# databricks/spark-deep-learning

Measured on AMD Instinct MI355X. Metric: images/sec, higher is better.
Workload: dtype bf16; 1 GPU; model=resnet50, global_batch=512, image=224, parallelism=dp1

## Files before the change

sparkdl/models/resnet.py:

```python

import torch
import torch.nn as nn

from sparkdl.ops import BatchNormAct2d, Conv1x1


class Bottleneck(nn.Module):
    expansion = 4

    def __init__(self, cin, width, stride=1):
        super().__init__()
        cout = width * self.expansion
        self.conv1 = Conv1x1(cin, width)
        self.bn1 = BatchNormAct2d(width, relu=True)
        self.conv2 = nn.Conv2d(width, width, 3, stride=stride, padding=1,
                               bias=False)
        self.bn2 = BatchNormAct2d(width, relu=True)
        self.conv3 = Conv1x1(width, cout)
        self.bn3 = BatchNormAct2d(cout, relu=True)
        if stride != 1 or cin != cout:
            self.down_conv = Conv1x1(cin, cout, stride=stride)
            self.down_bn = BatchNormAct2d(cout, relu=False)
        else:
            self.down_conv = None

    def forward(self, x):
        if self.down_conv is not None:
            idn = self.down_bn(self.down_conv(x))
        else:
            idn = x
        out = self.bn1(self.conv1(x))
        out = self.bn2(self.conv2(out))
        return self.bn3(self.conv3(out), residual=idn)


class ResNet50(nn.Module):
    LAYERS = (3, 4, 6, 3)

    def __init__(self, num_classes=1000):
        super().__init__()
        self.stem_conv = nn.Conv2d(3, 64, 7, stride=2, padding=3,
                                   bias=False)
        self.stem_bn = BatchNormAct2d(64, relu=True)
        self.stem_pool = nn.MaxPool2d(3, stride=2, padding=1)
        cin = 64
        stages = []
        for i, blocks in enumerate(self.LAYERS):
            width = 64 * (2 ** i)
            stride = 1 if i == 0 else 2
            layer = []
            for b in range(blocks):
                layer.append(Bottleneck(cin, width, stride if b == 0 else 1))
                cin = width * Bottleneck.expansion
            stages.append(nn.Sequential(*layer))
        self.stages = nn.Sequential(*stages)
        self.pool = nn.AdaptiveAvgPool2d(1)
        self.fc = nn.Linear(2048, num_classes)

        for m in self.modules():
            if isinstance(m, nn.Conv2d):
                nn.init.kaiming_normal_(m.weight, mode="fan_out",
                                        nonlinearity="relu")
        for m in self.modules():
            if isinstance(m, Bottleneck):
                nn.init.zeros_(m.bn3.weight)

    def forward(self, x):
        x = self.stem_pool(self.stem_bn(self.stem_conv(x)))
        x = self.stages(x)
        x = self.pool(x).flatten(1)
        return self.fc(x)
```

sparkdl/ops/__init__.py:

```python

_EXT = None
_EXT_ERR = None


def ext():
    global _EXT, _EXT_ERR
    if _EXT is None and _EXT_ERR is None:
        try:
            from sparkdl import _C
            _EXT = _C
        except ImportError as e:
            _EXT_ERR = e
    if _EXT is None:
        raise RuntimeError(
            "sparkdl._C HIP extension is not built. Run "
            "`python setup.py build_ext --inplace` (gfx950). "
            "Original error: %s" % _EXT_ERR)
    return _EXT


def has_ext():
    try:
        ext()
        return True
    except RuntimeError:
        return False


from sparkdl.ops.functional import (
    layer_norm, bias_gelu, batch_norm_act, layer_norm_ref, bias_gelu_ref,
    flash_attention, flash_attention_packed, masked_attention_ref,
    seqlens_from_mask,
)
from sparkdl.ops.modules import (
    LayerNorm, Linear, LinearGelu, Conv1x1, BatchNormAct2d,
    convert_bf16_training,
)
from sparkdl.ops.optim import FusedAdamW, FusedSGD
```

sparkdl/ops/csrc/batchnorm.hip:

```cpp

#include "common.hip.h"
#include "kernels.h"

namespace {

constexpr int kBlock = 256;
constexpr int kVec = 8;
constexpr int kUnroll = 2;
constexpr int kFoldFloats = kBlock * 2 * kVec;
constexpr int kFinCh = 4;


__device__ __forceinline__ void bn_store_pair(
    float* p, int cols, const float (&a)[kVec], const float (&b)[kVec]) {
  *(float4v*)(p) = float4v{a[0], a[1], a[2], a[3]};
  *(float4v*)(p + 4) = float4v{a[4], a[5], a[6], a[7]};
  *(float4v*)(p + cols) = float4v{b[0], b[1], b[2], b[3]};
  *(float4v*)(p + cols + 4) = float4v{b[4], b[5], b[6], b[7]};
}

__device__ __forceinline__ void bn_block_fold(
    float* lds, float (&a)[kVec], float (&b)[kVec], int rpb, int row_off,
    int lane_col, int cols, float* __restrict__ slab_row) {
  const bool active = row_off < rpb;
  float* mine = lds + (size_t)row_off * 2 * cols + lane_col;
  if (active) bn_store_pair(mine, cols, a, b);
  int s = 1;
  while (s < rpb) s <<= 1;
  int n = rpb;
  for (s >>= 1; s >= 1; s >>= 1) {
    __syncthreads();
    if (row_off < s && row_off + s < n) {
      const float* peer = mine + (size_t)s * 2 * cols;
      const float4v pa0 = *(const float4v*)(peer);
      const float4v pa1 = *(const float4v*)(peer + 4);
      const float4v pb0 = *(const float4v*)(peer + cols);
      const float4v pb1 = *(const float4v*)(peer + cols + 4);
#pragma unroll
      for (int j = 0; j < 4; ++j) {
        a[j] += pa0[j];
        a[j + 4] += pa1[j];
        b[j] += pb0[j];
        b[j + 4] += pb1[j];
      }
      if (s > 1) bn_store_pair(mine, cols, a, b);
    }
    n = min(n, s);
  }
  if (row_off == 0) bn_store_pair(slab_row + lane_col, cols, a, b);
}

__device__ __forceinline__ void bn_slab_sum(
    const float* __restrict__ slab, int G, int cols, int blk, float* red,
    float& sum_a, float& sum_b) {
  const int c = blk * kFinCh + threadIdx.x % kFinCh;
  float sa = 0.f, sb = 0.f;
#pragma unroll 4
  for (int g = threadIdx.x / kFinCh; g < G; g += kBlock / kFinCh) {
    const float* row = slab + (size_t)g * 2 * cols;
    sa += row[c];
    sb += row[cols + c];
  }
#pragma unroll
  for (int off = kFinCh; off < WAVE; off <<= 1) {
    sa += __shfl_xor(sa, off, WAVE);
    sb += __shfl_xor(sb, off, WAVE);
  }
  const int lane = threadIdx.x % WAVE;
  const int wid = threadIdx.x / WAVE;
  if (lane < kFinCh) {
    red[wid * 2 * kFinCh + lane] = sa;
    red[wid * 2 * kFinCh + kFinCh + lane] = sb;
  }
  __syncthreads();
  sum_a = 0.f;
  sum_b = 0.f;
  if (threadIdx.x < kFinCh) {
#pragma unroll
    for (int w = 0; w < kBlock / WAVE; ++w) {
      sum_a += red[w * 2 * kFinCh + threadIdx.x];
      sum_b += red[w * 2 * kFinCh + kFinCh + threadIdx.x];
    }
  }
}

__device__ __forceinline__ int bn_fin_block() {
  const int nb = gridDim.x;
  if (nb % 8) return blockIdx.x;
  return (blockIdx.x % 8) * (nb / 8) + blockIdx.x / 8;
}

template <int U>
__global__ __launch_bounds__(kBlock) void bn_stats_k(
// ... 16 lines not shown
        v[u] = *(const short8*)(x + (r + u * stride) * cols + lane_col);
#pragma unroll
      for (int u = 0; u < U; ++u) {
#pragma unroll
        for (int j = 0; j < kVec; ++j) {
          const float f = bf2f(v[u][j]);
          s[j] += f;
          ss[j] += f * f;
        }
      }
    }
    for (; r < rows; r += stride) {
      const short8 v = *(const short8*)(x + r * cols + lane_col);
#pragma unroll
      for (int j = 0; j < kVec; ++j) {
        const float f = bf2f(v[j]);
        s[j] += f;
        ss[j] += f * f;
      }
    }
  }
  bn_block_fold(lds, s, ss, rpb, row_off, lane_col, cols,
                slab + (size_t)blockIdx.x * 2 * cols);
}

__global__ __launch_bounds__(kBlock) void bn_finalize_k(
    const float* __restrict__ slab, int G, const float* __restrict__ gamma,
    const float* __restrict__ beta, float* __restrict__ running_mean,
    float* __restrict__ running_var, float* __restrict__ save_mean,
    float* __restrict__ save_rstd, float* __restrict__ scale,
    float* __restrict__ shift, long long rows, int cols, float momentum,
    float eps, int training) {
  __shared__ float red[kBlock / WAVE * 2 * kFinCh];
  float sum = 0.f, sumsq = 0.f;
  const int blk = bn_fin_block();
  if (training) bn_slab_sum(slab, G, cols, blk, red, sum, sumsq);
  if (threadIdx.x >= kFinCh) return;
  const int c = blk * kFinCh + threadIdx.x;
  float mean, rstd;
  if (training) {
    mean = sum / rows;
    const float var = fmaxf(sumsq / rows - mean * mean, 0.f);
    rstd = rsqrtf(var + eps);
    const float unbiased = rows > 1 ? var * rows / (rows - 1) : var;
    running_mean[c] += momentum * (mean - running_mean[c]);
    running_var[c] += momentum * (unbiased - running_var[c]);
    save_mean[c] = mean;
    save_rstd[c] = rstd;
  } else {
    mean = running_mean[c];
    rstd = rsqrtf(running_var[c] + eps);
    save_mean[c] = mean;
    save_rstd[c] = rstd;
  }
  const float sc = gamma[c] * rstd;
  scale[c] = sc;
  shift[c] = beta[c] - mean * sc;
}

template <bool RELU, bool RES>
__global__ __launch_bounds__(kBlock) void bn_apply_k(
    const short* __restrict__ x, const short* __restrict__ res,
    const float* __restrict__ scale, const float* __restrict__ shift,
    short* __restrict__ y, unsigned char* __restrict__ mask,
    long long rows, int cols) {
  const int tpr = cols / kVec;
  const int rpb = kBlock / min(tpr, kBlock);
  const int lane_col = (threadIdx.x % tpr) * kVec;
  const int row_off = threadIdx.x / tpr;
  if (row_off >= rpb) return;
  const float4v sc0 = *(const float4v*)(scale + lane_col);
  const float4v sc1 = *(const float4v*)(scale + lane_col + 4);
  const float4v sh0 = *(const float4v*)(shift + lane_col);
  const float4v sh1 = *(const float4v*)(shift + lane_col + 4);

  for (long long r = (long long)blockIdx.x * rpb + row_off; r < rows;
       r += (long long)gridDim.x * rpb) {
    const long long base = r * cols + lane_col;
    const short8 v = *(const short8*)(x + base);
    short8 o;
    unsigned char mbits = 0;
#pragma unroll
    for (int j = 0; j < kVec; ++j) {
      float f = bf2f(v[j]) * (j < 4 ? sc0[j] : sc1[j - 4]) +
                (j < 4 ? sh0[j] : sh1[j - 4]);
      if (RES) f += bf2f(res[base + j]);
      if (RELU) {
        if (f > 0.f) mbits |= (unsigned char)(1u << j);
        f = fmaxf(f, 0.f);
      }
      o[j] = f2bf(f);
    }
    *(short8*)(y + base) = o;
    if (RELU) mask[(r * cols + lane_col) / kVec] = mbits;
  }
}


template <bool RELU, int U>
__global__ __launch_bounds__(kBlock) void bn_bwd_reduce_k(
    const short* __restrict__ x, const unsigned char* __restrict__ mask,
    const short* __restrict__ dy, const float* __restrict__ save_mean,
    const float* __restrict__ save_rstd, float* __restrict__ slab,
    long long rows, int cols) {
  __shared__ __attribute__((aligned(16))) float lds[kFoldFloats];
  const int tpr = cols / kVec;
  const int rpb = kBlock / min(tpr, kBlock);
  const int lane_col = (threadIdx.x % tpr) * kVec;
  const int row_off = threadIdx.x / tpr;

  float s1[kVec] = {0.f}, s2[kVec] = {0.f};
  if (row_off < rpb) {
    const float4v m0 = *(const float4v*)(save_mean + lane_col);
    const float4v m1 = *(const float4v*)(save_mean + lane_col + 4);
    const float4v r0 = *(const float4v*)(save_rstd + lane_col);
    const float4v r1 = *(const float4v*)(save_rstd + lane_col + 4);
    auto accum = [&](const short8& xv, const short8& dv,
                     unsigned char mbits) {
#pragma unroll
      for (int j = 0; j < kVec; ++j) {
        float d = bf2f(dv[j]);
        if (RELU && !(mbits & (1u << j))) d = 0.f;
        const float mean = j < 4 ? m0[j] : m1[j - 4];
        const float rstd = j < 4 ? r0[j] : r1[j - 4];
        const float xh = (bf2f(xv[j]) - mean) * rstd;
        s1[j] += d;
        s2[j] += d * xh;
      }
    };
    const long long stride = (long long)gridDim.x * rpb;
    long long r = (long long)blockIdx.x * rpb + row_off;
    for (; r + (U - 1) * stride < rows; r += U * stride) {
      short8 xv[U], dv[U];
      unsigned char mb[U];
#pragma unroll
      for (int u = 0; u < U; ++u) {
        const long long base = (r + u * stride) * cols + lane_col;
        xv[u] = *(const short8*)(x + base);
        dv[u] = *(const short8*)(dy + base);
        mb[u] = 0xffu;
        if (RELU) mb[u] = mask[base / kVec];
      }
#pragma unroll
      for (int u = 0; u < U; ++u) accum(xv[u], dv[u], mb[u]);
    }
    for (; r < rows; r += stride) {
      const long long base = r * cols + lane_col;
      const short8 xv = *(const short8*)(x + base);
      const short8 dv = *(const short8*)(dy + base);
      unsigned char mbits = 0xffu;
      if (RELU) mbits = mask[base / kVec];
      accum(xv, dv, mbits);
    }
  }
  bn_block_fold(lds, s1, s2, rpb, row_off, lane_col, cols,
                slab + (size_t)blockIdx.x * 2 * cols);
}

__global__ __launch_bounds__(kBlock) void bn_bwd_finalize_k(
    const float* __restrict__ slab, int G, const float* __restrict__ gamma,
    const float* __restrict__ save_rstd, float* __restrict__ dgamma,
    float* __restrict__ dbeta, float* __restrict__ c1,
    float* __restrict__ c2, float* __restrict__ c3, long long rows,
    int cols, int training) {
  __shared__ float red[kBlock / WAVE * 2 * kFinCh];
  float sum_dym, sum_dymxh;
  const int blk = bn_fin_block();
  bn_slab_sum(slab, G, cols, blk, red, sum_dym, sum_dymxh);
  if (threadIdx.x >= kFinCh) return;
  const int c = blk * kFinCh + threadIdx.x;
  dgamma[c] = sum_dymxh;
  dbeta[c] = sum_dym;
  c1[c] = gamma[c] * save_rstd[c];
  if (training) {
    c2[c] = sum_dym / rows;
    c3[c] = sum_dymxh / rows;
  } else {
    c2[c] = 0.f;
    c3[c] = 0.f;
  }
}

template <bool RELU, bool RES>
__global__ __launch_bounds__(kBlock) void bn_bwd_apply_k(
    const short* __restrict__ x, const unsigned char* __restrict__ mask,
    const short* __restrict__ dy, const float* __restrict__ save_mean,
    const float* __restrict__ save_rstd, const float* __restrict__ c1,
    const float* __restrict__ c2, const float* __restrict__ c3,
    short* __restrict__ dx, short* __restrict__ dres, long long rows,
    int cols) {
  const int tpr = cols / kVec;
  const int rpb = kBlock / min(tpr, kBlock);
  const int lane_col = (threadIdx.x % tpr) * kVec;
  const int row_off = threadIdx.x / tpr;
  if (row_off >= rpb) return;
  const float4v m0 = *(const float4v*)(save_mean + lane_col);
  const float4v m1 = *(const float4v*)(save_mean + lane_col + 4);
  const float4v r0 = *(const float4v*)(save_rstd + lane_col);
  const float4v r1 = *(const float4v*)(save_rstd + lane_col + 4);
  const float4v a0 = *(const float4v*)(c1 + lane_col);
  const float4v a1 = *(const float4v*)(c1 + lane_col + 4);
  const float4v b0 = *(const float4v*)(c2 + lane_col);
  const float4v b1 = *(const float4v*)(c2 + lane_col + 4);
  const float4v g0 = *(const float4v*)(c3 + lane_col);
  const float4v g1 = *(const float4v*)(c3 + lane_col + 4);

  for (long long r = (long long)blockIdx.x * rpb + row_off; r < rows;
       r += (long long)gridDim.x * rpb) {
    const long long base = r * cols + lane_col;
    const short8 xv = *(const short8*)(x + base);
    const short8 dv = *(const short8*)(dy + base);
    unsigned char mbits = 0xffu;
    if (RELU) mbits = mask[base / kVec];
    short8 odx, odr;
#pragma unroll
    for (int j = 0; j < kVec; ++j) {
      float d = bf2f(dv[j]);
      if (RELU && !(mbits & (1u << j))) d = 0.f;
      const float mean = j < 4 ? m0[j] : m1[j - 4];
      const float rstd = j < 4 ? r0[j] : r1[j - 4];
      const float xh = (bf2f(xv[j]) - mean) * rstd;
      const float k1 = j < 4 ? a0[j] : a1[j - 4];
      const float k2 = j < 4 ? b0[j] : b1[j - 4];
      const float k3 = j < 4 ? g0[j] : g1[j - 4];
      odx[j] = f2bf(k1 * (d - k2 - xh * k3));
      if (RES) odr[j] = f2bf(d);
    }
    *(short8*)(dx + base) = odx;
    if (RES) *(short8*)(dres + base) = odr;
  }
}

int bn_grid(long long rows, int cols) {
  const int tpr = cols / kVec;
  const int rpb = kBlock / min(tpr, kBlock);
  long long blocks = (rows + rpb - 1) / rpb;
  return (int)min(blocks, 2048LL);
}

}

int bn_reduce_blocks(long long rows, int cols) {
  const int tpr = cols / kVec;
  const int rpb = kBlock / min(tpr, kBlock);
  const long long row_blocks = (rows + rpb - 1) / rpb;
  const long long g = max(256LL, min(512LL, rows / 64));
  return (int)max(1LL, min(row_blocks, g));
}

long long bn_scratch_floats(long long rows, int cols) {
  return (long long)bn_reduce_blocks(rows, cols) * 2 * cols + 3LL * cols;
}

void launch_bn_fwd(const short* x, const short* res, const float* gamma,
                   const float* beta, float* running_mean,
                   float* running_var, float* save_mean, float* save_rstd,
                   float* scratch, short* y, unsigned char* mask,
                   long long rows, int cols, float momentum, float eps,
                   bool training, bool relu, hipStream_t stream) {
  const int grid = bn_grid(rows, cols);
  const int G = bn_reduce_blocks(rows, cols);
  if (training)
    hipLaunchKernelGGL(bn_stats_k<kUnroll>, dim3(G), dim3(kBlock), 0,
                       stream, x, scratch, rows, cols);
  float* scale = scratch + (size_t)G * 2 * cols;
  float* shift = scale + cols;
  hipLaunchKernelGGL(bn_finalize_k, dim3(cols / kFinCh), dim3(kBlock), 0,
                     stream, scratch, G, gamma, beta, running_mean,
                     running_var, save_mean, save_rstd, scale, shift, rows,
                     cols, momentum, eps, (int)training);
  auto ap = relu ? (res ? bn_apply_k<true, true> : bn_apply_k<true, false>)
                 : (res ? bn_apply_k<false, true>
                        : bn_apply_k<false, false>);
  hipLaunchKernelGGL(ap, dim3(grid), dim3(kBlock), 0, stream, x, res,
                     scale, shift, y, mask, rows, cols);
}

void launch_bn_bwd(const short* x, const unsigned char* mask,
                   const short* dy, const float* gamma,
                   const float* save_mean, const float* save_rstd,
                   float* scratch, float* dgamma, float* dbeta, short* dx,
                   short* dres, long long rows, int cols, bool training,
                   bool relu, hipStream_t stream) {
  const int grid = bn_grid(rows, cols);
  const int G = bn_reduce_blocks(rows, cols);
  auto rk = relu ? bn_bwd_reduce_k<true, kUnroll>
                 : bn_bwd_reduce_k<false, kUnroll>;
  hipLaunchKernelGGL(rk, dim3(G), dim3(kBlock), 0, stream, x, mask, dy,
                     save_mean, save_rstd, scratch, rows, cols);
  float* c1 = scratch + (size_t)G * 2 * cols;
  float* c2 = c1 + cols;
  float* c3 = c2 + cols;
  hipLaunchKernelGGL(bn_bwd_finalize_k, dim3(cols / kFinCh), dim3(kBlock),
                     0, stream, scratch, G, gamma, save_rstd, dgamma, dbeta,
                     c1, c2, c3, rows, cols, (int)training);
  auto ak = relu ? (dres ? bn_bwd_apply_k<true, true>
                         : bn_bwd_apply_k<true, false>)
                 : (dres ? bn_bwd_apply_k<false, true>
                         : bn_bwd_apply_k<false, false>);
  hipLaunchKernelGGL(ak, dim3(grid), dim3(kBlock), 0, stream, x, mask, dy,
                     save_mean, save_rstd, c1, c2, c3, dx, dres, rows,
                     cols);
}
```

sparkdl/ops/csrc/bindings.cpp:

```cpp

#include <torch/extension.h>
#include <ATen/hip/impl/HIPStreamMasqueradingAsCUDA.h>
#include <ATen/hip/impl/HIPGuardImplMasqueradingAsCUDA.h>

#include <cmath>
#include <vector>

#include "kernels.h"

namespace {

using DeviceGuard = c10::hip::HIPGuardMasqueradingAsCUDA;

hipStream_t cur_stream() {
  return c10::hip::getCurrentHIPStreamMasqueradingAsCUDA().stream();
}

#define CHECK_BF16_CUDA(t)                                            \
  TORCH_CHECK((t).is_cuda(), #t " must be on GPU");                   \
  TORCH_CHECK((t).scalar_type() == at::kBFloat16, #t " must be bf16");\
  TORCH_CHECK((t).is_contiguous(), #t " must be contiguous")

#define CHECK_F32_CUDA(t)                                             \
  TORCH_CHECK((t).is_cuda(), #t " must be on GPU");                   \
// ... 103 lines not shown
      dgamma.data_ptr<float>(), dbeta.data_ptr<float>(), ws_rows, cols,
      cur_stream());
  return {dx, dgamma, dbeta};
}


std::vector<at::Tensor> bn_fwd(const at::Tensor& x,
                               const c10::optional<at::Tensor>& res,
                               const at::Tensor& gamma,
                               const at::Tensor& beta,
                               at::Tensor running_mean,
                               at::Tensor running_var, double momentum,
                               double eps, bool training, bool relu) {
  CHECK_BF16_CUDA(x);
  CHECK_F32_CUDA(gamma);
  CHECK_F32_CUDA(beta);
  DeviceGuard guard(x.device());
  const int cols = (int)x.size(-1);
  const long long rows = x.numel() / cols;
  TORCH_CHECK(cols % 8 == 0 && cols <= 2048,
              "bn_fwd requires cols%8==0 and cols<=2048 (NHWC channels)");
  const short* res_ptr = nullptr;
  if (res.has_value()) {
    CHECK_BF16_CUDA(res.value());
    TORCH_CHECK(res->sizes() == x.sizes());
    res_ptr = bf_ptr(res.value());
  }
  auto f32 = x.options().dtype(at::kFloat);
  auto y = at::empty_like(x);
  auto save_mean = at::empty({cols}, f32);
  auto save_rstd = at::empty({cols}, f32);
  auto scratch = at::empty({bn_scratch_floats(rows, cols)}, f32);
  at::Tensor mask;
  unsigned char* mask_ptr = nullptr;
  if (relu) {
    mask = at::empty({rows * cols / 8}, x.options().dtype(at::kByte));
    mask_ptr = mask.data_ptr<unsigned char>();
  } else {
    mask = at::empty({0}, x.options().dtype(at::kByte));
  }
  launch_bn_fwd(bf_ptr(x), res_ptr, gamma.data_ptr<float>(),
                beta.data_ptr<float>(), running_mean.data_ptr<float>(),
                running_var.data_ptr<float>(), save_mean.data_ptr<float>(),
                save_rstd.data_ptr<float>(), scratch.data_ptr<float>(),
                bf_ptr_mut(y), mask_ptr, rows, cols, (float)momentum,
                (float)eps, training, relu, cur_stream());
  return {y, save_mean, save_rstd, mask};
}

std::vector<at::Tensor> bn_bwd(const at::Tensor& x,
                               const at::Tensor& mask,
                               const at::Tensor& dy,
                               const at::Tensor& gamma,
                               const at::Tensor& save_mean,
                               const at::Tensor& save_rstd, bool training,
                               bool relu, bool needs_dres) {
  CHECK_BF16_CUDA(x);
  CHECK_BF16_CUDA(dy);
  CHECK_F32_CUDA(gamma);
  DeviceGuard guard(x.device());
  const int cols = (int)x.size(-1);
  const long long rows = x.numel() / cols;
  TORCH_CHECK(!relu || mask.numel() == rows * cols / 8,
              "relu backward needs the forward's activation mask");
  auto f32 = x.options().dtype(at::kFloat);
  auto dx = at::empty_like(x);
  auto dgamma = at::empty({cols}, f32);
  auto dbeta = at::empty({cols}, f32);
  auto scratch = at::empty({bn_scratch_floats(rows, cols)}, f32);
  at::Tensor dres;
  short* dres_ptr = nullptr;
  if (needs_dres) {
    dres = at::empty_like(x);
    dres_ptr = bf_ptr_mut(dres);
  }
  launch_bn_bwd(bf_ptr(x),
                relu ? mask.data_ptr<unsigned char>() : nullptr,
                bf_ptr(dy), gamma.data_ptr<float>(),
                save_mean.data_ptr<float>(), save_rstd.data_ptr<float>(),
                scratch.data_ptr<float>(), dgamma.data_ptr<float>(),
                dbeta.data_ptr<float>(), bf_ptr_mut(dx), dres_ptr, rows,
                cols, training, relu, cur_stream());
  if (needs_dres) return {dx, dgamma, dbeta, dres};
  return {dx, dgamma, dbeta};
}


at::Tensor bias_gelu_fwd(const at::Tensor& x, const at::Tensor& bias) {
  CHECK_BF16_CUDA(x);
  CHECK_F32_CUDA(bias);
  DeviceGuard guard(x.device());
  const int cols = (int)x.size(-1);
  const long long rows = x.numel() / cols;
  TORCH_CHECK(bias.numel() == cols);
  auto y = at::empty_like(x);
  launch_bias_gelu_fwd(bf_ptr(x), bias.data_ptr<float>(), bf_ptr_mut(y),
                       rows, cols, cur_stream());
  return y;
}

std::vector<at::Tensor> bias_gelu_bwd(const at::Tensor& x,
                                      const at::Tensor& bias,
                                      const at::Tensor& dy) {
  CHECK_BF16_CUDA(x);
  CHECK_BF16_CUDA(dy);
  CHECK_F32_CUDA(bias);
  DeviceGuard guard(x.device());
  const int cols = (int)x.size(-1);
  const long long rows = x.numel() / cols;
  TORCH_CHECK(cols <= 16384, "bias_gelu_bwd LDS partials support cols<=16384");
  auto dx = at::empty_like(x);
  auto dbias = at::zeros({cols}, x.options().dtype(at::kFloat));
  launch_bias_gelu_bwd(bf_ptr(x), bias.data_ptr<float>(), bf_ptr(dy),
                       bf_ptr_mut(dx), dbias.data_ptr<float>(), rows, cols,
                       cur_stream());
  return {dx, dbias};
}


std::vector<at::Tensor> gemm_bias_act(const at::Tensor& A,
                                      const at::Tensor& W,
                                      const c10::optional<at::Tensor>& bias,
                                      int64_t act, bool save_z) {
  CHECK_BF16_CUDA(A);
  CHECK_BF16_CUDA(W);
  TORCH_CHECK(A.dim() == 2 && W.dim() == 2 && A.size(1) == W.size(1));
  const int M = (int)A.size(0), K = (int)A.size(1), N = (int)W.size(0);
  TORCH_CHECK(gemm_bias_act_supported(M, N, K),
              "gemm_bias_act requires K % 64 == 0");
  const float* bias_ptr = nullptr;
  if (bias.has_value()) {
    CHECK_F32_CUDA(bias.value());
    TORCH_CHECK(bias->numel() == N);
    bias_ptr = bias->data_ptr<float>();
  }
  DeviceGuard guard(A.device());
  auto C = at::empty({M, N}, A.options());
  at::Tensor Z;
  short* z_ptr = nullptr;
  if (save_z && act != 0) {
    Z = at::empty({M, N}, A.options());
    z_ptr = bf_ptr_mut(Z);
  }
  launch_gemm_bias_act(bf_ptr(A), bf_ptr(W), bias_ptr, bf_ptr_mut(C),
                       z_ptr, M, N, K, (int)act, cur_stream());
  if (z_ptr) return {C, Z};
  return {C};
}

at::Tensor gemm_stream(const at::Tensor& A, const at::Tensor& W) {
  CHECK_BF16_CUDA(A);
  CHECK_BF16_CUDA(W);
  TORCH_CHECK(A.dim() == 2 && W.dim() == 2 && A.size(1) == W.size(1));
  const long long M = A.size(0);
  const int K = (int)A.size(1), N = (int)W.size(0);
  TORCH_CHECK(gemm_stream_supported(M, N, K),
              "gemm_stream requires K in {64,128,256} and N % 64 == 0");
  DeviceGuard guard(A.device());
  auto C = at::empty({M, N}, A.options());
  launch_gemm_stream(bf_ptr(A), bf_ptr(W), bf_ptr_mut(C), M, N, K,
                     cur_stream());
  return C;
}


static const long long* seed_ptr(const c10::optional<at::Tensor>& seed) {
// ... 161 lines not shown
}

at::Tensor wgrad_splitk(const at::Tensor& dZ, const at::Tensor& X) {
  CHECK_BF16_CUDA(dZ);
  CHECK_BF16_CUDA(X);
  TORCH_CHECK(dZ.dim() == 2 && X.dim() == 2 && dZ.size(0) == X.size(0));
  const long long M = dZ.size(0);
  const int N = (int)dZ.size(1), K = (int)X.size(1);
  TORCH_CHECK(wgrad_splitk_supported(M, N, K),
              "wgrad_splitk requires N%256==0, K%128==0, M%64==0");
  DeviceGuard guard(dZ.device());
  auto dW = at::empty({N, K}, dZ.options().dtype(at::kFloat));
  launch_wgrad_splitk(bf_ptr(dZ), bf_ptr(X), dW.data_ptr<float>(), M, N,
                      K, cur_stream());
  return dW;
}

at::Tensor transpose_bf16(const at::Tensor& X) {
  CHECK_BF16_CUDA(X);
  TORCH_CHECK(X.dim() == 2 && X.is_contiguous());
  DeviceGuard guard(X.device());
  const int R = (int)X.size(0), C = (int)X.size(1);
  auto Y = at::empty({C, R}, X.options());
  launch_transpose_bf16(bf_ptr(X), bf_ptr_mut(Y), R, C, cur_stream());
  return Y;
}


at::Tensor gbt_histogram(const at::Tensor& B, const at::Tensor& g,
                         const at::Tensor& h, const at::Tensor& row_list,
                         const at::Tensor& bmap, int64_t n_nodes) {
  TORCH_CHECK(B.is_cuda() && B.scalar_type() == at::kByte &&
              B.is_contiguous());
  CHECK_F32_CUDA(g);
  CHECK_F32_CUDA(h);
  TORCH_CHECK(row_list.is_cuda() && row_list.scalar_type() == at::kInt);
  TORCH_CHECK(bmap.is_cuda() && bmap.scalar_type() == at::kInt &&
              bmap.size(-1) == 4);
  DeviceGuard guard(B.device());
  const int F = (int)B.size(1);
  TORCH_CHECK(F % 8 == 0, "feature dim must be padded to a multiple of 8");
  auto hist = at::zeros({n_nodes, F, 256, 2},
                        B.options().dtype(at::kFloat));
  launch_gbt_histogram(
      B.data_ptr<unsigned char>(), g.data_ptr<float>(),
      h.data_ptr<float>(), row_list.data_ptr<int>(),
      reinterpret_cast<const int4*>(bmap.data_ptr<int>()),
      (int)(bmap.numel() / 4), F, hist.data_ptr<float>(), cur_stream());
  return hist;
}

}

PYBIND11_MODULE(TORCH_EXTENSION_NAME, m) {
  m.doc() = "sparkdl MI355X-native kernels (gfx950)";
  m.def("fused_adamw_", &fused_adamw_, "Fused multi-tensor AdamW step");
  m.def("fused_sgd_", &fused_sgd_, "Fused multi-tensor SGD step");
  m.def("zero_grads_", &zero_grads_, "Zero all grads in a chunk table");
  m.def("gemm_bias_act", &gemm_bias_act, "MFMA GEMM + bias(+GELU) (N6)");
  m.def("transpose_bf16", &transpose_bf16, "bf16 2D transpose (dgrad W^T)");
  m.def("gemm_stream", &gemm_stream,
        "Streaming tall-skinny GEMM (1x1 convs)");
  m.def("wgrad_splitk", &wgrad_splitk,
        "Split-M wgrad GEMM (tr_b16 fragment path)");
  m.def("attn_fwd", &attn_fwd, "Flash attention fwd (D=64, bf16)",
        py::arg("q"), py::arg("k"), py::arg("v"), py::arg("dropout_p"),
        py::arg("seed"), py::arg("seqlens") = py::none());
  m.def("attn_bwd", &attn_bwd, "Flash attention bwd (dQ/dK/dV)",
        py::arg("q"), py::arg("k"), py::arg("v"), py::arg("dO"),
        py::arg("lse"), py::arg("drow"), py::arg("dropout_p"),
        py::arg("seed"), py::arg("seqlens") = py::none());
  m.def("attn_fwd_packed", &attn_fwd_packed,
        "Flash attention fwd over the packed qkv buffer", py::arg("qkv"),
        py::arg("dropout_p"), py::arg("seed"),
        py::arg("seqlens") = py::none());
  m.def("attn_bwd_packed", &attn_bwd_packed,
        "Flash attention bwd -> packed dqkv", py::arg("qkv"),
        py::arg("dO"), py::arg("lse"), py::arg("drow"),
        py::arg("dropout_p"), py::arg("seed"),
        py::arg("seqlens") = py::none());
  m.def("gbt_histogram", &gbt_histogram, "GBT g/h histogram (N7)");
  m.def("bn_fwd", &bn_fwd, "Fused BatchNorm(+add)(+ReLU) fwd (bf16 NHWC)");
  m.def("bn_bwd", &bn_bwd, "Fused BatchNorm(+add)(+ReLU) bwd (bf16 NHWC)");
  m.def("layernorm_fwd", &layernorm_fwd, "LayerNorm forward (bf16)");
  m.def("layernorm_bwd", &layernorm_bwd, "LayerNorm backward (bf16)");
  m.def("bias_gelu_fwd", &bias_gelu_fwd, "Fused bias+GELU forward (bf16)");
  m.def("bias_gelu_bwd", &bias_gelu_bwd, "Fused bias+GELU backward (bf16)");
  m.attr("_chunk_elems") = kOptChunk;
}
```

sparkdl/ops/csrc/kernels.h:

```cpp
#pragma once

#include <hip/hip_runtime.h>
#include <cstdint>

struct TensorChunk {
  float* p;
  const float* g;
  float* m;
  float* v;
  long long n;
  short* pl;
};

constexpr int kOptChunk = 16384;

void launch_fused_adamw(const TensorChunk* chunks, const int2* bmap,
                        int nblocks, float lr, float beta1, float beta2,
                        float eps, float weight_decay,
                        long long* step_counter, float* coeffs,
                        hipStream_t stream);

void launch_fused_sgd(const TensorChunk* chunks, const int2* bmap,
                      int nblocks, float lr, float momentum,
                      float weight_decay, bool nesterov, bool first_step,
                      hipStream_t stream);

void launch_layernorm_fwd(const short* x, const float* gamma,
                          const float* beta, short* y, float* save_mean,
                          float* save_rstd, int rows, int cols, float eps,
                          hipStream_t stream);

void launch_layernorm_bwd(const short* x, const short* dy,
                          const float* gamma, const float* save_mean,
                          const float* save_rstd, short* dx,
                          float* dgamma_part, float* dbeta_part,
                          int part_rows, int rows, int cols,
                          hipStream_t stream);

int layernorm_bwd_part_rows(int rows);

void launch_layernorm_reduce_parts(const float* dgamma_part,
                                   const float* dbeta_part, float* dgamma,
                                   float* dbeta, int part_rows, int cols,
                                   hipStream_t stream);

void launch_bias_gelu_fwd(const short* x, const float* bias, short* y,
                          long long rows, int cols, hipStream_t stream);

void launch_bias_gelu_bwd(const short* x, const float* bias,
                          const short* dy, short* dx, float* dbias,
                          long long rows, int cols, hipStream_t stream);

int bn_reduce_blocks(long long rows, int cols);
long long bn_scratch_floats(long long rows, int cols);

void launch_bn_fwd(const short* x, const short* res, const float* gamma,
                   const float* beta, float* running_mean,
                   float* running_var, float* save_mean, float* save_rstd,
                   float* scratch, short* y, unsigned char* mask,
                   long long rows, int cols, float momentum, float eps,
                   bool training, bool relu, hipStream_t stream);

void launch_bn_bwd(const short* x, const unsigned char* mask,
                   const short* dy, const float* gamma,
                   const float* save_mean, const float* save_rstd,
                   float* scratch, float* dgamma, float* dbeta, short* dx,
                   short* dres, long long rows, int cols, bool training,
                   bool relu, hipStream_t stream);

void launch_gemm_bias_act(const short* A, const short* W,
                          const float* bias, short* C, short* Z, int M,
                          int N, int K, int act, hipStream_t stream);
bool gemm_bias_act_supported(int M, int N, int K);

void launch_gemm_stream(const short* A, const short* W, short* C,
                        long long M, int N, int K, hipStream_t stream);
bool gemm_stream_supported(long long M, int N, int K);

void launch_wgrad_splitk(const short* dZ, const short* X, float* dW,
                         long long M, int N, int K, hipStream_t stream);
bool wgrad_splitk_supported(long long M, int N, int K);

void launch_transpose_bf16(const short* X, short* Y, int R, int C,
                           hipStream_t stream);

void launch_attn_pretranspose(const short* X, short* T, int BH, int S,
                              int H, int rs, hipStream_t stream);
void launch_attn_fwd(const short* Q, const short* K, const short* VT,
                     short* O, float* LSE, const long long* seed, int BH,
                     int S, int H, int rs, int ors, float dropout_p,
                     const int* seqlens, hipStream_t stream);
void launch_attn_bwd(const short* Q, const short* K, const short* V,
                     const short* dO, const short* QT, const short* DOT,
                     const short* KT, const float* LSE, const float* Drow,
                     short* dQ, short* dK, short* dV,
                     const long long* seed, int BH, int S, int H, int rs,
                     int ors, int grs, float dropout_p,
                     const int* seqlens, hipStream_t stream);

void launch_gbt_histogram(const unsigned char* B, const float* g,
                          const float* h, const int* row_list,
                          const int4* bmap, int nblocks, int F,
                          float* hist, hipStream_t stream);

void launch_zero_grads(const TensorChunk* chunks, const int2* bmap,
                       int nblocks, hipStream_t stream);
```

sparkdl/ops/functional.py:

```python

import os

import torch

import sparkdl.ops as _ops



def layer_norm_ref(x, gamma, beta, eps=1e-5):
    xf = x.float()
    out = torch.nn.functional.layer_norm(
        xf, (x.shape[-1],), gamma.float(), beta.float(), eps)
    return out.to(x.dtype)


def bias_gelu_ref(x, bias):
    return torch.nn.functional.gelu(
        x.float() + bias.float(), approximate="none").to(x.dtype)


def masked_attention_ref(q, k, v, seq_lens, dropout_p=0.0):
    S, d = q.shape[-2], q.shape[-1]
    qf, kf, vf = q.float(), k.float(), v.float()
    lens = torch.as_tensor(seq_lens, device=q.device).clamp(0, S)
# ... 39 lines not shown
        C = _ops.ext()
        x = x.contiguous()
        y, mean, rstd = C.layernorm_fwd(x, gamma, beta, eps)
        ctx.save_for_backward(x, gamma, mean, rstd)
        return y

    @staticmethod
    def backward(ctx, dy):
        C = _ops.ext()
        x, gamma, mean, rstd = ctx.saved_tensors
        dx, dgamma, dbeta = C.layernorm_bwd(
            x, dy.contiguous(), gamma, mean, rstd)
        return dx, dgamma, dbeta, None


class _BiasGeluFn(torch.autograd.Function):
    @staticmethod
    def forward(ctx, x, bias):
        C = _ops.ext()
        x = x.contiguous()
        ctx.save_for_backward(x, bias)
        return C.bias_gelu_fwd(x, bias)

    @staticmethod
    def backward(ctx, dy):
        C = _ops.ext()
        x, bias = ctx.saved_tensors
        dx, dbias = C.bias_gelu_bwd(x, bias, dy.contiguous())
        return dx, dbias


def _to_nhwc(t):
    return t.permute(0, 2, 3, 1).contiguous(memory_format=torch.contiguous_format)


def _from_nhwc(t):
    return t.permute(0, 3, 1, 2)


class _BNReLUFn(torch.autograd.Function):
    @staticmethod
    def forward(ctx, x, residual, gamma, beta, running_mean, running_var,
                momentum, eps, training, relu):
        C = _ops.ext()
        xp = _to_nhwc(x)
        rp = _to_nhwc(residual) if residual is not None else None
        y, mean, rstd, mask = C.bn_fwd(
            xp, rp, gamma, beta, running_mean, running_var, momentum,
            eps, training, relu)
        ctx.save_for_backward(xp, mask, gamma, mean, rstd)
        ctx.bn_flags = (training, relu, residual is not None)
        return _from_nhwc(y)

    @staticmethod
    def backward(ctx, dy):
        C = _ops.ext()
        xp, mask, gamma, mean, rstd = ctx.saved_tensors
        training, relu, has_res = ctx.bn_flags
        needs_dres = has_res and ctx.needs_input_grad[1]
        outs = C.bn_bwd(xp, mask, _to_nhwc(dy), gamma, mean, rstd,
                        training, relu, needs_dres)
        dx = _from_nhwc(outs[0])
        dres = _from_nhwc(outs[3]) if needs_dres else None
        return (dx, dres, outs[1], outs[2], None, None, None, None, None,
                None)


def batch_norm_act(x, gamma, beta, running_mean, running_var,
                   momentum=0.1, eps=1e-5, training=True, relu=False,
                   residual=None):
    C = x.shape[1]
    if (x.is_cuda and x.dtype == torch.bfloat16
            and C <= 2048 and C % 8 == 0):
        return _BNReLUFn.apply(x, residual, gamma, beta, running_mean,
                               running_var, momentum, eps, training, relu)
    y = torch.nn.functional.batch_norm(
        x.float(), running_mean, running_var, gamma, beta,
        training, momentum, eps).to(x.dtype)
    if residual is not None:
        y = y + residual
    return torch.relu(y) if relu else y


def layer_norm(x, gamma, beta, eps=1e-5):
    if x.is_cuda and x.dtype == torch.bfloat16:
        return _LayerNormFn.apply(x, gamma, beta, eps)
    return torch.nn.functional.layer_norm(
        x, (x.shape[-1],), gamma.to(x.dtype), beta.to(x.dtype), eps)


def bias_gelu(x, bias):
    if x.is_cuda and x.dtype == torch.bfloat16:
        return _BiasGeluFn.apply(x, bias)
    return torch.nn.functional.gelu(x + bias.to(x.dtype), approximate="none")



_zero_bias_cache = {}


def _zero_bias(n, device):
    key = (n, device)
    if key not in _zero_bias_cache:
        _zero_bias_cache[key] = torch.zeros(
            n, dtype=torch.float32, device=device)
    return _zero_bias_cache[key]


class _LinearGeluFusedFn(torch.autograd.Function):

    @staticmethod
    def forward(ctx, x2d, weight, bias):
        C = _ops.ext()
        y, z = C.gemm_bias_act(x2d, weight, bias, 1, True)
        ctx.save_for_backward(x2d, weight, z)
        return y

    @staticmethod
    def backward(ctx, dy):
        C = _ops.ext()
        x2d, weight, z = ctx.saved_tensors
        dy = dy.contiguous()
        dz, dbias = C.bias_gelu_bwd(z, _zero_bias(z.shape[-1], z.device),
                                    dy)
        if (weight.shape[0] % 64 == 0
                and os.environ.get("SPARKDL_FUSED_DGRAD", "1") != "0"):
            wt = C.transpose_bf16(weight)
            dx = C.gemm_bias_act(dz, wt, None, 0, False)[0]
        else:
            dx = dz @ weight
        dw = _wgrad(dz, x2d)
        return dx, dw, dbias


def linear_gelu_fused(x, weight, bias):
    shape = x.shape
    x2d = x.reshape(-1, shape[-1]).contiguous()
    y = _LinearGeluFusedFn.apply(x2d, weight.contiguous(), bias)
    return y.reshape(*shape[:-1], weight.shape[0])


def linear_gelu_fused_ok(x, weight):
    return (x.is_cuda and x.dtype == torch.bfloat16
            and weight.dtype == torch.bfloat16
            and x.shape[-1] % 64 == 0)



_attn_seed = {}


def _attn_seed_tensor(device):
    if device not in _attn_seed:
        rank = int(os.environ.get("RANK", "0"))
        _attn_seed[device] = torch.randint(
            0, 2 ** 31, (1,), dtype=torch.int64,
            device=device) + rank * 2654435761 % (2 ** 31)
    return _attn_seed[device]


class _FlashAttnFn(torch.autograd.Function):

    @staticmethod
    def forward(ctx, q, k, v, dropout_p, seq_lens=None):
        C = _ops.ext()
        seed = None
# ... 171 lines not shown
```

Measured before the change: 9427 images/s.

## Fuse stem BatchNorm, ReLU and MaxPool into one forward and backward kernel

Adds HIP kernels that apply the stem BatchNorm affine and ReLU and compute the 3x3 stride-2 max pool in one pass. Each output stores a per-channel byte tap code so backward can route pooled gradients straight into the BN backward reduce and apply kernels. This avoids writing and re-reading the full-resolution BN/ReLU activation and separate max-pool kernels in both directions. The cost is recomputing the affine transform for overlapping windows (9 loads per output) and gathering up to four pooled gradients per input pixel in backward.

```diff
diff --git a/sparkdl/models/resnet.py b/sparkdl/models/resnet.py
--- a/sparkdl/models/resnet.py
+++ b/sparkdl/models/resnet.py
@@ -2,7 +2,7 @@
 import torch
 import torch.nn as nn
 
-from sparkdl.ops import BatchNormAct2d, Conv1x1
+from sparkdl.ops import BatchNormAct2d, Conv1x1, batch_norm_relu_maxpool
 
 
 class Bottleneck(nn.Module):
@@ -66,7 +66,11 @@
                 nn.init.zeros_(m.bn3.weight)
 
     def forward(self, x):
-        x = self.stem_pool(self.stem_bn(self.stem_conv(x)))
+        bn = self.stem_bn
+        x = batch_norm_relu_maxpool(
+            self.stem_conv(x), bn.weight, bn.bias, bn.running_mean,
+            bn.running_var, momentum=bn.momentum, eps=bn.eps,
+            training=bn.training)
         x = self.stages(x)
         x = self.pool(x).flatten(1)
         return self.fc(x)
diff --git a/sparkdl/ops/__init__.py b/sparkdl/ops/__init__.py
--- a/sparkdl/ops/__init__.py
+++ b/sparkdl/ops/__init__.py
@@ -28,7 +28,8 @@
 
 
 from sparkdl.ops.functional import (
-    layer_norm, bias_gelu, batch_norm_act, layer_norm_ref, bias_gelu_ref,
+    layer_norm, bias_gelu, batch_norm_act, batch_norm_relu_maxpool,
+    layer_norm_ref, bias_gelu_ref,
     flash_attention, flash_attention_packed, masked_attention_ref,
     seqlens_from_mask,
 )
diff --git a/sparkdl/ops/csrc/batchnorm.hip b/sparkdl/ops/csrc/batchnorm.hip
--- a/sparkdl/ops/csrc/batchnorm.hip
+++ b/sparkdl/ops/csrc/batchnorm.hip
@@ -9,6 +9,18 @@
 constexpr int kUnroll = 2;
 constexpr int kFoldFloats = kBlock * 2 * kVec;
 constexpr int kFinCh = 4;
+
+__device__ __forceinline__ float bn_affine(short x, float scale,
+                                           float shift) {
+  return bf2f(x) * scale + shift;
+}
+__device__ __forceinline__ float bn_xhat(short x, float mean, float rstd) {
+  return (bf2f(x) - mean) * rstd;
+}
+__device__ __forceinline__ float bn_dx(float d, float xh, float k1,
+                                       float k2, float k3) {
+  return k1 * (d - k2 - xh * k3);
+}
 
 
 __device__ __forceinline__ void bn_store_pair(
@@ -191,8 +203,8 @@
     unsigned char mbits = 0;
 #pragma unroll
     for (int j = 0; j < kVec; ++j) {
-      float f = bf2f(v[j]) * (j < 4 ? sc0[j] : sc1[j - 4]) +
-                (j < 4 ? sh0[j] : sh1[j - 4]);
+      float f = bn_affine(v[j], j < 4 ? sc0[j] : sc1[j - 4],
+                          j < 4 ? sh0[j] : sh1[j - 4]);
       if (RES) f += bf2f(res[base + j]);
       if (RELU) {
         if (f > 0.f) mbits |= (unsigned char)(1u << j);
@@ -232,7 +244,7 @@
         if (RELU && !(mbits & (1u << j))) d = 0.f;
         const float mean = j < 4 ? m0[j] : m1[j - 4];
         const float rstd = j < 4 ? r0[j] : r1[j - 4];
-        const float xh = (bf2f(xv[j]) - mean) * rstd;
+        const float xh = bn_xhat(xv[j], mean, rstd);
         s1[j] += d;
         s2[j] += d * xh;
       }
@@ -328,15 +340,257 @@
       if (RELU && !(mbits & (1u << j))) d = 0.f;
       const float mean = j < 4 ? m0[j] : m1[j - 4];
       const float rstd = j < 4 ? r0[j] : r1[j - 4];
-      const float xh = (bf2f(xv[j]) - mean) * rstd;
+      const float xh = bn_xhat(xv[j], mean, rstd);
       const float k1 = j < 4 ? a0[j] : a1[j - 4];
       const float k2 = j < 4 ? b0[j] : b1[j - 4];
       const float k3 = j < 4 ? g0[j] : g1[j - 4];
-      odx[j] = f2bf(k1 * (d - k2 - xh * k3));
+      odx[j] = f2bf(bn_dx(d, xh, k1, k2, k3));
       if (RES) odr[j] = f2bf(d);
     }
     *(short8*)(dx + base) = odx;
     if (RES) *(short8*)(dres + base) = odr;
+  }
+}
+
+
+typedef unsigned uint2v __attribute__((ext_vector_type(2)));
+
+constexpr unsigned kPoolDead = 9;
+constexpr unsigned kPoolNone = 0xffu;
+
+struct PoolGeom {
+  int H, W, Ho, Wo;
+};
+
+__global__ __launch_bounds__(kBlock) void bn_apply_pool_k(
+    const short* __restrict__ x, const float* __restrict__ scale,
+    const float* __restrict__ shift, short* __restrict__ pooled,
+    unsigned char* __restrict__ code, long long orows, int cols,
+    PoolGeom g) {
+  const int tpr = cols / kVec;
+  const int rpb = kBlock / min(tpr, kBlock);
+  const int lane_col = (threadIdx.x % tpr) * kVec;
+  const int row_off = threadIdx.x / tpr;
+  if (row_off >= rpb) return;
+  const float4v sc0 = *(const float4v*)(scale + lane_col);
+  const float4v sc1 = *(const float4v*)(scale + lane_col + 4);
+  const float4v sh0 = *(const float4v*)(shift + lane_col);
+  const float4v sh1 = *(const float4v*)(shift + lane_col + 4);
+  const unsigned opix = (unsigned)(g.Ho * g.Wo);
+
+  for (long long o = (long long)blockIdx.x * rpb + row_off; o < orows;
+       o += (long long)gridDim.x * rpb) {
+    const unsigned n = (unsigned)o / opix;
+    const unsigned rem = (unsigned)o - n * opix;
+    const int oh = (int)(rem / (unsigned)g.Wo);
+    const int ow = (int)(rem - (unsigned)oh * (unsigned)g.Wo);
+    short8 v[9];
+#pragma unroll
+    for (int kh = 0; kh < 3; ++kh) {
+      const int ih = min(max(2 * oh - 1 + kh, 0), g.H - 1);
+#pragma unroll
+      for (int kw = 0; kw < 3; ++kw) {
+        const int iw = min(max(2 * ow - 1 + kw, 0), g.W - 1);
+        const long long r = ((long long)n * g.H + ih) * g.W + iw;
+        v[kh * 3 + kw] = *(const short8*)(x + r * cols + lane_col);
+      }
+    }
+    float best[kVec], bestf[kVec];
+    unsigned tap[kVec];
+#pragma unroll
+    for (int j = 0; j < kVec; ++j) {
+      best[j] = -INFINITY;
+      bestf[j] = 0.f;
+      tap[j] = 0;
+    }
+#pragma unroll
+    for (int kh = 0; kh < 3; ++kh) {
+      const int ih = 2 * oh - 1 + kh;
+      const bool hin = ih >= 0 && ih < g.H;
+#pragma unroll
+      for (int kw = 0; kw < 3; ++kw) {
+        const int iw = 2 * ow - 1 + kw;
+        const bool in = hin && iw >= 0 && iw < g.W;
+#pragma unroll
+        for (int j = 0; j < kVec; ++j) {
+          const float f =
+              bn_affine(v[kh * 3 + kw][j], j < 4 ? sc0[j] : sc1[j - 4],
+                        j < 4 ? sh0[j] : sh1[j - 4]);
+          const float q = bf2f(f2bf(fmaxf(f, 0.f)));
+          if (in && q > best[j]) {
+            best[j] = q;
+            bestf[j] = f;
+            tap[j] = kh * 3 + kw;
+          }
+        }
+      }
+    }
+    short8 ov;
+    unsigned c0 = 0, c1 = 0;
+#pragma unroll
+    for (int j = 0; j < kVec; ++j) {
+      union { float f; unsigned u; } b;
+      b.f = best[j];
+      ov[j] = (short)(b.u >> 16);
+      const unsigned c = bestf[j] > 0.f ? tap[j] : kPoolDead;
+      if (j < 4) c0 |= c << (8 * j);
+      else c1 |= c << (8 * (j - 4));
+    }
+    const long long base = o * cols + lane_col;
+    *(short8*)(pooled + base) = ov;
+    *(uint2v*)(code + base) = uint2v{c0, c1};
+  }
+}
+
+struct PoolTaps {
+  short8 dy[4];
+  uint2v code[4];
+  unsigned want[4];
+};
+
+__device__ __forceinline__ PoolTaps bn_pool_taps(
+    const short* __restrict__ dyp, const unsigned char* __restrict__ code,
+    long long r, int cols, int lane_col, const PoolGeom& g) {
+  const unsigned ipix = (unsigned)(g.H * g.W);
+  const unsigned n = (unsigned)r / ipix;
+  const unsigned rem = (unsigned)r - n * ipix;
+  const int ih = (int)(rem / (unsigned)g.W);
+  const int iw = (int)(rem - (unsigned)ih * (unsigned)g.W);
+  const int oh0 = ih >> 1, ow0 = iw >> 1;
+  const unsigned kh0 = 1 + (ih & 1), kw0 = 1 + (iw & 1);
+  const bool h2 = (ih & 1) && oh0 + 1 < g.Ho;
+  const bool w2 = (iw & 1) && ow0 + 1 < g.Wo;
+  PoolTaps t;
+#pragma unroll
+  for (int a = 0; a < 2; ++a) {
+#pragma unroll
+    for (int b = 0; b < 2; ++b) {
+      const bool on = (a == 0 || h2) && (b == 0 || w2);
+      const int oh = on ? oh0 + a : oh0;
+      const int ow = on ? ow0 + b : ow0;
+      const long long base =
+          (((long long)n * g.Ho + oh) * g.Wo + ow) * cols + lane_col;
+      t.dy[a * 2 + b] = *(const short8*)(dyp + base);
+      t.code[a * 2 + b] = *(const uint2v*)(code + base);
+      t.want[a * 2 + b] =
+          on ? (a ? 0u : kh0) * 3 + (b ? 0u : kw0) : kPoolNone;
+    }
+  }
+  return t;
+}
+
+__device__ __forceinline__ void bn_pool_dym(const PoolTaps& t,
+                                            float (&d)[kVec]) {
+#pragma unroll
+  for (int j = 0; j < kVec; ++j) d[j] = 0.f;
+#pragma unroll
+  for (int w = 0; w < 4; ++w) {
+#pragma unroll
+    for (int j = 0; j < kVec; ++j) {
+      const unsigned c =
+          ((j < 4 ? t.code[w][0] : t.code[w][1]) >> (8 * (j & 3))) & 0xffu;
+      if (c == t.want[w]) d[j] += bf2f(t.dy[w][j]);
+    }
+  }
+#pragma unroll
+  for (int j = 0; j < kVec; ++j) d[j] = bf2f(f2bf(d[j]));
+}
+
+template <int U>
+__global__ __launch_bounds__(kBlock) void bn_pool_bwd_reduce_k(
+    const short* __restrict__ x, const unsigned char* __restrict__ code,
+    const short* __restrict__ dyp, const float* __restrict__ save_mean,
+    const float* __restrict__ save_rstd, float* __restrict__ slab,
+    long long rows, int cols, PoolGeom g) {
+  __shared__ __attribute__((aligned(16))) float lds[kFoldFloats];
+  const int tpr = cols / kVec;
+  const int rpb = kBlock / min(tpr, kBlock);
+  const int lane_col = (threadIdx.x % tpr) * kVec;
+  const int row_off = threadIdx.x / tpr;
+
+  float s1[kVec] = {0.f}, s2[kVec] = {0.f};
+  if (row_off < rpb) {
+    const float4v m0 = *(const float4v*)(save_mean + lane_col);
+    const float4v m1 = *(const float4v*)(save_mean + lane_col + 4);
+    const float4v r0 = *(const float4v*)(save_rstd + lane_col);
+    const float4v r1 = *(const float4v*)(save_rstd + lane_col + 4);
+    auto accum = [&](const short8& xv, const PoolTaps& t) {
+      float d[kVec];
+      bn_pool_dym(t, d);
+#pragma unroll
+      for (int j = 0; j < kVec; ++j) {
+        const float mean = j < 4 ? m0[j] : m1[j - 4];
+        const float rstd = j < 4 ? r0[j] : r1[j - 4];
+        const float xh = bn_xhat(xv[j], mean, rstd);
+        s1[j] += d[j];
+        s2[j] += d[j] * xh;
+      }
+    };
+    const long long stride = (long long)gridDim.x * rpb;
+    long long r = (long long)blockIdx.x * rpb + row_off;
+    for (; r + (U - 1) * stride < rows; r += U * stride) {
+      short8 xv[U];
+      PoolTaps t[U];
+#pragma unroll
+      for (int u = 0; u < U; ++u) {
+        const long long ru = r + u * stride;
+        xv[u] = *(const short8*)(x + ru * cols + lane_col);
+        t[u] = bn_pool_taps(dyp, code, ru, cols, lane_col, g);
+      }
+#pragma unroll
+      for (int u = 0; u < U; ++u) accum(xv[u], t[u]);
+    }
+    for (; r < rows; r += stride) {
+      const short8 xv = *(const short8*)(x + r * cols + lane_col);
+      const PoolTaps t = bn_pool_taps(dyp, code, r, cols, lane_col, g);
+      accum(xv, t);
+    }
+  }
+  bn_block_fold(lds, s1, s2, rpb, row_off, lane_col, cols,
+                slab + (size_t)blockIdx.x * 2 * cols);
+}
+
+__global__ __launch_bounds__(kBlock) void bn_pool_bwd_apply_k(
+    const short* __restrict__ x, const unsigned char* __restrict__ code,
+    const short* __restrict__ dyp, const float* __restrict__ save_mean,
+    const float* __restrict__ save_rstd, const float* __restrict__ c1,
+    const float* __restrict__ c2, const float* __restrict__ c3,
+    short* __restrict__ dx, long long rows, int cols, PoolGeom g) {
+  const int tpr = cols / kVec;
+  const int rpb = kBlock / min(tpr, kBlock);
+  const int lane_col = (threadIdx.x % tpr) * kVec;
+  const int row_off = threadIdx.x / tpr;
+  if (row_off >= rpb) return;
+  const float4v m0 = *(const float4v*)(save_mean + lane_col);
+  const float4v m1 = *(const float4v*)(save_mean + lane_col + 4);
+  const float4v r0 = *(const float4v*)(save_rstd + lane_col);
+  const float4v r1 = *(const float4v*)(save_rstd + lane_col + 4);
+  const float4v a0 = *(const float4v*)(c1 + lane_col);
+  const float4v a1 = *(const float4v*)(c1 + lane_col + 4);
+  const float4v b0 = *(const float4v*)(c2 + lane_col);
+  const float4v b1 = *(const float4v*)(c2 + lane_col + 4);
+  const float4v g0 = *(const float4v*)(c3 + lane_col);
+  const float4v g1 = *(const float4v*)(c3 + lane_col + 4);
+
+  for (long long r = (long long)blockIdx.x * rpb + row_off; r < rows;
+       r += (long long)gridDim.x * rpb) {
+    const long long base = r * cols + lane_col;
+    const short8 xv = *(const short8*)(x + base);
+    const PoolTaps t = bn_pool_taps(dyp, code, r, cols, lane_col, g);
+    float d[kVec];
+    bn_pool_dym(t, d);
+    short8 odx;
+#pragma unroll
+    for (int j = 0; j < kVec; ++j) {
+      const float mean = j < 4 ? m0[j] : m1[j - 4];
+      const float rstd = j < 4 ? r0[j] : r1[j - 4];
+      const float xh = bn_xhat(xv[j], mean, rstd);
+      const float k1 = j < 4 ? a0[j] : a1[j - 4];
+      const float k2 = j < 4 ? b0[j] : b1[j - 4];
+      const float k3 = j < 4 ? g0[j] : g1[j - 4];
+      odx[j] = f2bf(bn_dx(d[j], xh, k1, k2, k3));
+    }
+    *(short8*)(dx + base) = odx;
   }
 }
 
@@ -411,3 +665,51 @@
                      save_mean, save_rstd, c1, c2, c3, dx, dres, rows,
                      cols);
 }
+
+void launch_bn_pool_fwd(const short* x, const float* gamma,
+                        const float* beta, float* running_mean,
+                        float* running_var, float* save_mean,
+                        float* save_rstd, float* scratch, short* pooled,
+                        unsigned char* code, int n, int h, int w, int cols,
+                        float momentum, float eps, bool training,
+                        hipStream_t stream) {
+  const PoolGeom g{h, w, (h - 1) / 2 + 1, (w - 1) / 2 + 1};
+  const long long rows = (long long)n * h * w;
+  const long long orows = (long long)n * g.Ho * g.Wo;
+  const int G = bn_reduce_blocks(rows, cols);
+  if (training)
+    hipLaunchKernelGGL(bn_stats_k<kUnroll>, dim3(G), dim3(kBlock), 0,
+                       stream, x, scratch, rows, cols);
+  float* scale = scratch + (size_t)G * 2 * cols;
+  float* shift = scale + cols;
+  hipLaunchKernelGGL(bn_finalize_k, dim3(cols / kFinCh), dim3(kBlock), 0,
+                     stream, scratch, G, gamma, beta, running_mean,
+                     running_var, save_mean, save_rstd, scale, shift, rows,
+                     cols, momentum, eps, (int)training);
+  hipLaunchKernelGGL(bn_apply_pool_k, dim3(bn_grid(orows, cols)),
+                     dim3(kBlock), 0, stream, x, scale, shift, pooled, code,
+                     orows, cols, g);
+}
+
+void launch_bn_pool_bwd(const short* x, const unsigned char* code,
+                        const short* dyp, const float* gamma,
+                        const float* save_mean, const float* save_rstd,
+                        float* scratch, float* dgamma, float* dbeta,
+                        short* dx, int n, int h, int w, int cols,
+                        bool training, hipStream_t stream) {
+  const PoolGeom g{h, w, (h - 1) / 2 + 1, (w - 1) / 2 + 1};
+  const long long rows = (long long)n * h * w;
+  const int G = bn_reduce_blocks(rows, cols);
+  hipLaunchKernelGGL(bn_pool_bwd_reduce_k<kUnroll>, dim3(G), dim3(kBlock),
+                     0, stream, x, code, dyp, save_mean, save_rstd, scratch,
+                     rows, cols, g);
+  float* c1 = scratch + (size_t)G * 2 * cols;
+  float* c2 = c1 + cols;
+  float* c3 = c2 + cols;
+  hipLaunchKernelGGL(bn_bwd_finalize_k, dim3(cols / kFinCh), dim3(kBlock),
+                     0, stream, scratch, G, gamma, save_rstd, dgamma, dbeta,
+                     c1, c2, c3, rows, cols, (int)training);
+  hipLaunchKernelGGL(bn_pool_bwd_apply_k, dim3(bn_grid(rows, cols)),
+                     dim3(kBlock), 0, stream, x, code, dyp, save_mean,
+                     save_rstd, c1, c2, c3, dx, rows, cols, g);
+}
diff --git a/sparkdl/ops/csrc/bindings.cpp b/sparkdl/ops/csrc/bindings.cpp
--- a/sparkdl/ops/csrc/bindings.cpp
+++ b/sparkdl/ops/csrc/bindings.cpp
@@ -209,6 +209,90 @@
                 dbeta.data_ptr<float>(), bf_ptr_mut(dx), dres_ptr, rows,
                 cols, training, relu, cur_stream());
   if (needs_dres) return {dx, dgamma, dbeta, dres};
+  return {dx, dgamma, dbeta};
+}
+
+std::vector<at::Tensor> bn_pool_fwd(const at::Tensor& x,
+                                    const at::Tensor& gamma,
+                                    const at::Tensor& beta,
+                                    at::Tensor running_mean,
+                                    at::Tensor running_var, double momentum,
+                                    double eps, bool training) {
+  CHECK_BF16_CUDA(x);
+  CHECK_F32_CUDA(gamma);
+  CHECK_F32_CUDA(beta);
+  CHECK_F32_CUDA(running_mean);
+  CHECK_F32_CUDA(running_var);
+  TORCH_CHECK(x.dim() == 4, "bn_pool_fwd takes x as [N,H,W,C]");
+  DeviceGuard guard(x.device());
+  const int64_t n = x.size(0), h = x.size(1), w = x.size(2);
+  const int cols = (int)x.size(3);
+  TORCH_CHECK(cols % 8 == 0 && cols <= 2048,
+              "bn_pool_fwd requires cols%8==0 and cols<=2048");
+  TORCH_CHECK(n > 0 && h > 0 && w > 0 && n * h * w < (1LL << 31),
+              "bn_pool_fwd requires 0 < N*H*W < 2^31");
+  TORCH_CHECK(gamma.numel() == cols && beta.numel() == cols &&
+              running_mean.numel() == cols && running_var.numel() == cols);
+  const int64_t ho = (h - 1) / 2 + 1, wo = (w - 1) / 2 + 1;
+  auto f32 = x.options().dtype(at::kFloat);
+  auto pooled = at::empty({n, ho, wo, cols}, x.options());
+  auto code = at::empty({n, ho, wo, cols}, x.options().dtype(at::kByte));
+  auto save_mean = at::empty({cols}, f32);
+  auto save_rstd = at::empty({cols}, f32);
+  auto scratch = at::empty({bn_scratch_floats(n * h * w, cols)}, f32);
+  launch_bn_pool_fwd(bf_ptr(x), gamma.data_ptr<float>(),
+                     beta.data_ptr<float>(), running_mean.data_ptr<float>(),
+                     running_var.data_ptr<float>(),
+                     save_mean.data_ptr<float>(),
+                     save_rstd.data_ptr<float>(), scratch.data_ptr<float>(),
+                     bf_ptr_mut(pooled), code.data_ptr<unsigned char>(),
+                     (int)n, (int)h, (int)w, cols, (float)momentum,
+                     (float)eps, training, cur_stream());
+  return {pooled, save_mean, save_rstd, code};
+}
+
+std::vector<at::Tensor> bn_pool_bwd(const at::Tensor& x,
+                                    const at::Tensor& code,
+                                    const at::Tensor& dyp,
+                                    const at::Tensor& gamma,
+                                    const at::Tensor& save_mean,
+                                    const at::Tensor& save_rstd,
+                                    bool training) {
+  CHECK_BF16_CUDA(x);
+  CHECK_BF16_CUDA(dyp);
+  CHECK_F32_CUDA(gamma);
+  CHECK_F32_CUDA(save_mean);
+  CHECK_F32_CUDA(save_rstd);
+  TORCH_CHECK(x.dim() == 4, "bn_pool_bwd takes x as [N,H,W,C]");
+  DeviceGuard guard(x.device());
+  const int64_t n = x.size(0), h = x.size(1), w = x.size(2);
+  const int cols = (int)x.size(3);
+  TORCH_CHECK(cols % 8 == 0 && cols <= 2048,
+              "bn_pool_bwd requires cols%8==0 and cols<=2048");
+  TORCH_CHECK(n > 0 && h > 0 && w > 0 && n * h * w < (1LL << 31),
+              "bn_pool_bwd requires 0 < N*H*W < 2^31");
+  const int64_t ho = (h - 1) / 2 + 1, wo = (w - 1) / 2 + 1;
+  const std::vector<int64_t> pshape = {n, ho, wo, (int64_t)cols};
+  TORCH_CHECK(dyp.sizes() == at::IntArrayRef(pshape),
+              "pooled grad must be [N,Ho,Wo,C]");
+  TORCH_CHECK(code.is_cuda() && code.scalar_type() == at::kByte &&
+              code.is_contiguous() &&
+              code.sizes() == at::IntArrayRef(pshape),
+              "backward needs the forward's tap codes");
+  TORCH_CHECK(gamma.numel() == cols && save_mean.numel() == cols &&
+              save_rstd.numel() == cols);
+  auto f32 = x.options().dtype(at::kFloat);
+  auto dx = at::empty_like(x);
+  auto dgamma = at::empty({cols}, f32);
+  auto dbeta = at::empty({cols}, f32);
+  auto scratch = at::empty({bn_scratch_floats(n * h * w, cols)}, f32);
+  launch_bn_pool_bwd(bf_ptr(x), code.data_ptr<unsigned char>(),
+                     bf_ptr(dyp), gamma.data_ptr<float>(),
+                     save_mean.data_ptr<float>(),
+                     save_rstd.data_ptr<float>(), scratch.data_ptr<float>(),
+                     dgamma.data_ptr<float>(), dbeta.data_ptr<float>(),
+                     bf_ptr_mut(dx), (int)n, (int)h, (int)w, cols, training,
+                     cur_stream());
   return {dx, dgamma, dbeta};
 }
 
@@ -536,6 +620,10 @@
   m.def("gbt_histogram", &gbt_histogram, "GBT g/h histogram (N7)");
   m.def("bn_fwd", &bn_fwd, "Fused BatchNorm(+add)(+ReLU) fwd (bf16 NHWC)");
   m.def("bn_bwd", &bn_bwd, "Fused BatchNorm(+add)(+ReLU) bwd (bf16 NHWC)");
+  m.def("bn_pool_fwd", &bn_pool_fwd,
+        "Fused BatchNorm+ReLU+MaxPool(3,2,1) fwd (bf16 NHWC)");
+  m.def("bn_pool_bwd", &bn_pool_bwd,
+        "Fused BatchNorm+ReLU+MaxPool(3,2,1) bwd (bf16 NHWC)");
   m.def("layernorm_fwd", &layernorm_fwd, "LayerNorm forward (bf16)");
   m.def("layernorm_bwd", &layernorm_bwd, "LayerNorm backward (bf16)");
   m.def("bias_gelu_fwd", &bias_gelu_fwd, "Fused bias+GELU forward (bf16)");
diff --git a/sparkdl/ops/csrc/kernels.h b/sparkdl/ops/csrc/kernels.h
--- a/sparkdl/ops/csrc/kernels.h
+++ b/sparkdl/ops/csrc/kernels.h
@@ -68,6 +68,21 @@
                    short* dres, long long rows, int cols, bool training,
                    bool relu, hipStream_t stream);
 
+void launch_bn_pool_fwd(const short* x, const float* gamma,
+                        const float* beta, float* running_mean,
+                        float* running_var, float* save_mean,
+                        float* save_rstd, float* scratch, short* pooled,
+                        unsigned char* code, int n, int h, int w, int cols,
+                        float momentum, float eps, bool training,
+                        hipStream_t stream);
+
+void launch_bn_pool_bwd(const short* x, const unsigned char* code,
+                        const short* dyp, const float* gamma,
+                        const float* save_mean, const float* save_rstd,
+                        float* scratch, float* dgamma, float* dbeta,
+                        short* dx, int n, int h, int w, int cols,
+                        bool training, hipStream_t stream);
+
 void launch_gemm_bias_act(const short* A, const short* W,
                           const float* bias, short* C, short* Z, int M,
                           int N, int K, int act, hipStream_t stream);
diff --git a/sparkdl/ops/functional.py b/sparkdl/ops/functional.py
--- a/sparkdl/ops/functional.py
+++ b/sparkdl/ops/functional.py
@@ -145,6 +145,44 @@
     return torch.relu(y) if relu else y
 
 
+class _BNReLUPoolFn(torch.autograd.Function):
+
+    @staticmethod
+    def forward(ctx, x, gamma, beta, running_mean, running_var, momentum,
+                eps, training):
+        C = _ops.ext()
+        xp = _to_nhwc(x)
+        pooled, mean, rstd, code = C.bn_pool_fwd(
+            xp, gamma, beta, running_mean, running_var, momentum, eps,
+            training)
+        ctx.save_for_backward(xp, code, gamma, mean, rstd)
+        ctx.bn_training = training
+        return _from_nhwc(pooled)
+
+    @staticmethod
+    def backward(ctx, dy):
+        C = _ops.ext()
+        xp, code, gamma, mean, rstd = ctx.saved_tensors
+        dx, dgamma, dbeta = C.bn_pool_bwd(
+            xp, code, _to_nhwc(dy), gamma, mean, rstd, ctx.bn_training)
+        return _from_nhwc(dx), dgamma, dbeta, None, None, None, None, None
+
+
+def batch_norm_relu_maxpool(x, gamma, beta, running_mean, running_var,
+                            momentum=0.1, eps=1e-5, training=True):
+    C = x.shape[1]
+    if (x.is_cuda and x.dtype == torch.bfloat16 and x.dim() == 4
+            and C <= 2048 and C % 8 == 0
+            and 0 < x.numel() // C < 2 ** 31
+            and os.environ.get("SPARKDL_FUSED_STEM", "1") != "0"):
+        return _BNReLUPoolFn.apply(x, gamma, beta, running_mean,
+                                   running_var, momentum, eps, training)
+    y = batch_norm_act(x, gamma, beta, running_mean, running_var,
+                       momentum=momentum, eps=eps, training=training,
+                       relu=True)
+    return torch.nn.functional.max_pool2d(y, 3, stride=2, padding=1)
+
+
 def layer_norm(x, gamma, beta, eps=1e-5):
     if x.is_cuda and x.dtype == torch.bfloat16:
         return _LayerNormFn.apply(x, gamma, beta, eps)
```

Result: faster. 9705 images/s, median of 6 (+3.0%).
